# google-research/Splat-SLAM

Hardware: AMD Instinct MI355X
Metric: mapping frames/sec + render ms @640x480, 300k Gaussians; PSNR vs ref (higher is better)
Workload: dtype f32

## Files before the change

### include/splat_hip.h

```cpp
#ifndef SPLAT_HIP_H_
#define SPLAT_HIP_H_

#include <stddef.h>
#include <stdint.h>

#ifdef __cplusplus
extern "C" {
#endif

#define SGR_ABI_VERSION 10

typedef enum SgrStatus {
  SGR_OK = 0,
  SGR_ERR_INVALID = -1,
  SGR_ERR_WORKSPACE = -2,
  SGR_ERR_CAPACITY = -3,
  SGR_ERR_HIP = -4
} SgrStatus;

typedef struct SgrSettings {
  int32_t num_gaussians;
  int32_t image_height;
  int32_t image_width;
  int32_t sh_degree;
// ... 83 lines not shown
} SgrBackwardView;
int sgr_backward_views(int32_t num_views, const SgrBackwardView* views, const SgrInputs* in, const SgrGradInputs* grad_in,
                       void* stream);

int sgr_densify_stats(int64_t n, const float* dL_dmeans2D, const int32_t* radii, float* stat_grad_accum, float* stat_denom,
                      float* stat_max_radii, void* stream);

int sgr_query(const void* saved, int64_t* num_rendered_host, int32_t* overflow_host, void* stream);

int sgr_query_header(const void* saved, uint32_t words_host[16], void* stream);

int sgr_header_to_host(const void* saved, void* pinned_host64, void* stream);

int sgr_query_stats(const SgrWorkspace* ws, int32_t num_gaussians, int32_t image_height, int32_t image_width,
                    const int32_t* radii, int64_t stats_host[4], void* stream);
int sgr_query_depth_keys(const SgrWorkspace* ws, int32_t num_gaussians, int32_t image_height, int32_t image_width,
                         const int32_t* radii, float* depth_out, void* stream);
int sgr_query_list_histogram(const SgrWorkspace* ws, int32_t num_gaussians, int32_t image_height, int32_t image_width,
                             int64_t hist_host[8], void* stream);

#define SGR_OPT_FUSED_BLEND 0
#define SGR_OPT_UPSTREAM_POSE_JACOBIAN 1
#define SGR_OPT_SEGMENT_TEST 2
#define SGR_OPT_COUNT 3
int sgr_set_option(int32_t option, int32_t value);
int sgr_get_option(int32_t option);

#define SGR_PROFILE_KINDS 7
int sgr_profile_enable(uint32_t kind_mask);
int sgr_profile_read(float ms_host[SGR_PROFILE_KINDS], int64_t launches_host[SGR_PROFILE_KINDS]);

int sgr_mapping_loss(int32_t H, int32_t W, const float* image, const float* depth,
                     const float* gt_image, const float* gt_depth,
                     const float* exposure_a, const float* exposure_b,
                     float alpha, float rgb_boundary_threshold, float upstream,
                     float* loss, float* dL_dimage, float* dL_ddepth, float* dL_dexp_a, float* dL_dexp_b,
                     void* scratch, size_t scratch_bytes, void* stream);

size_t sgr_ssim_scratch_bytes(int32_t B, int32_t C, int32_t H, int32_t W);
int sgr_ssim(int32_t B, int32_t C, int32_t H, int32_t W, const float* img1, const float* img2, float* ssim_out, float* maps,
             void* scratch, size_t scratch_bytes, void* stream);
int sgr_ssim_backward(int32_t B, int32_t C, int32_t H, int32_t W, const float* img1, const float* img2, const float* maps,
                      const float* upstream, int32_t upstream_stride, float upstream_scale, float* dL_dimg1, void* stream);

typedef struct SgrMetricFrame {
  const float* render;
  const float* gt_image;
// ... 485 lines not shown
```

### splat_slam_amd/_native.py

```python
import ctypes as C
import os

_HERE = os.path.dirname(os.path.abspath(__file__))
LIB_PATH = os.environ.get("SPLAT_HIP_LIB") or os.path.join(_HERE, "lib", "libsplat_hip.so")

SGR_OPT_FUSED_BLEND = 0
SGR_OPT_UPSTREAM_POSE_JACOBIAN = 1
SGR_OPT_SEGMENT_TEST = 2
SGR_OK, SGR_ERR_INVALID, SGR_ERR_WORKSPACE, SGR_ERR_CAPACITY, SGR_ERR_HIP = 0, -1, -2, -3, -4

_fp = C.c_void_p


class SgrSettings(C.Structure):
    _fields_ = [("num_gaussians", C.c_int32), ("image_height", C.c_int32), ("image_width", C.c_int32),
                ("sh_degree", C.c_int32), ("sh_coeffs", C.c_int32), ("tanfovx", C.c_float), ("tanfovy", C.c_float),
                ("scale_modifier", C.c_float), ("prefiltered", C.c_int32), ("debug", C.c_int32),
                ("bg", _fp), ("viewmatrix", _fp), ("projmatrix", _fp), ("projmatrix_raw", _fp), ("campos", _fp)]


class SgrInputs(C.Structure):
    _fields_ = [("means3D", _fp), ("opacities", _fp), ("shs", _fp), ("colors_precomp", _fp), ("scales", _fp),
                ("rotations", _fp), ("cov3D_precomp", _fp)]


class SgrOutputs(C.Structure):
    _fields_ = [("color", _fp), ("depth", _fp), ("opacity", _fp), ("radii", _fp), ("n_touched", _fp)]


class SgrWorkspace(C.Structure):
    _fields_ = [("saved", _fp), ("saved_bytes", C.c_size_t), ("scratch", _fp), ("scratch_bytes", C.c_size_t),
# ... 350 lines not shown
```

### splat_slam_amd/csrc/sgr_api.hip

```cpp
#include <cstdarg>
#include <cstdio>
#include <cstring>
#include <cstdlib>
#include <vector>

#include <hip/hip_runtime.h>

#include "sgr_common.h"

namespace sgr {

void launch_preprocess_fwd(const ViewTab&, int, const LOff&, const Common&, const SgrInputs&, hipStream_t);
void launch_preprocess_bwd(const ViewTab&, int, const LOff&, const Common&, const SgrInputs&, const SgrGradInputs&, const FusedAdam*,
                           hipStream_t, bool mapping_loop = false);
void launch_binning(const ViewTab&, int, const LOff&, hipStream_t);
void launch_zero_heads(const ViewTab&, int, const LOff&, size_t, hipStream_t);
void launch_blend_fwd(const ViewTab&, int, const LOff&, const float*, const LossTab*, const LossCoef*, hipStream_t);
void launch_blend_bwd(const ViewTab&, int, const LOff&, const float*, const LossTab*, const LossCoef*, hipStream_t);
void launch_blend_fused(const ViewTab&, int, const LOff&, const float*, const LossTab&, const LossCoef&, hipStream_t);
bool blend_can_fuse(const LOff&);

static int g_opt[SGR_OPT_COUNT] = {1, 0, 0};

static thread_local char g_err[512] = "";
int set_error(int code, const char* fmt, ...) {
  va_list ap;
  va_start(ap, fmt);
  vsnprintf(g_err, sizeof(g_err), fmt, ap);
  va_end(ap);
  return code;
}
#define HIP_TRY(expr)                                                                                   \
  do {                                                                                                  \
    hipError_t _e = (expr);                                                                             \
    if (_e != hipSuccess) return set_error(SGR_ERR_HIP, "%s failed: %s", #expr, hipGetErrorString(_e)); \
  } while (0)

int debug_flags() {
  static int f = -1;
  if (f < 0) { const char* e = getenv("SGR_DEBUG"); f = e ? atoi(e) : 0; }
  return f | (g_opt[SGR_OPT_SEGMENT_TEST] ? 0 : 4);
}

static Layout make_layout(int N, int H, int W, int64_t cap) { return Layout(N, H, W, cap); }

// ... 268 lines not shown
  for (int base = 0; base < num_views; base += kMaxViews) {
    const int nv = num_views - base < kMaxViews ? num_views - base : kMaxViews;
    ViewTab tab = {};
    for (int v = 0; v < nv; ++v) {
      const SgrBackwardView& m = views[base + v];
      if (int rc = check_workspace(&m.ws, L)) return rc;
      tab_set_view(tab, v, &m.settings, nullptr, &m.ws);
      tab.radii[v] = const_cast<int32_t*>(m.radii);
      tab.dL_dcolor[v] = m.dL_dcolor; tab.dL_ddepth[v] = m.dL_ddepth; tab.dL_dtau[v] = m.dL_dtau; tab.dL_dmeans2D[v] = m.dL_dmeans2D;
    }
    SgrGradInputs gv = g;
    gv.accumulate = (grad_in->accumulate || base > 0) ? 1 : 0;
    launch_blend_bwd(tab, nv, d, f.settings.bg, nullptr, nullptr, st);
    launch_preprocess_bwd(tab, nv, d, cm, *in, gv, nullptr, st);
  }
  HIP_TRY(hipGetLastError());
  return SGR_OK;
}

}

static int map_views_impl(int32_t num_views, const SgrMapView* views, const SgrInputs* in, const SgrGradInputs* grads, float alpha,
                          float rgb_boundary_threshold, int32_t forward_only, FusedAdam* fused, bool* fused_done,
                          void* stream, bool store_sinks = false, const SgrSsimTerm* term = nullptr) {
  if (fused_done) *fused_done = false;
  if (num_views < 0 || (num_views > 0 && (!views || !in)) || (!forward_only && !grads))
    return set_error(SGR_ERR_INVALID, "map_views: null argument");
  if (num_views == 0) return SGR_OK;
  if (forward_only) term = nullptr;
  if (term) {
    if (!term->arena || term->max_views <= 0)
      return set_error(SGR_ERR_INVALID, "map_views: SSIM term without an arena");
    for (int v = 0; v < num_views; ++v) {
      const SgrMapView& m = views[v];
      const int H = m.settings.image_height, W = m.settings.image_width;
      if (!m.out.color || !m.out.depth || !m.out.opacity)
        return set_error(SGR_ERR_INVALID, "map_views: the SSIM loss needs every view's rendered image, depth and opacity");
      if (term->arena_bytes < sgr_ssim_term_bytes(term->max_views, H, W))
        return set_error(SGR_ERR_WORKSPACE, "map_views: SSIM arena too small (need %zu for %d views of %dx%d)",
                         sgr_ssim_term_bytes(term->max_views, H, W), term->max_views, W, H);
      if (!m.loss_scratch || m.loss_scratch_bytes < (size_t)ssim_loss_nparts(H, W) * sizeof(LossPart))
        return set_error(SGR_ERR_WORKSPACE, "map_views: loss_scratch too small for the SSIM loss (need %zu)",
                         (size_t)ssim_loss_nparts(H, W) * sizeof(LossPart));
    }
  }
  hipStream_t st = (hipStream_t)stream;
  bool uniform = true;
// ... 33 lines not shown
                                           mv.loss, mv.dL_dimage, mv.dL_ddepth, mv.dL_dexposure,
                                           mv.dL_dexposure ? mv.dL_dexposure + 1 : nullptr, stream))
          return rc;
      } else if (int rc = sgr_mapping_loss(mv.settings.image_height, mv.settings.image_width, mv.out.color, mv.out.depth, mv.gt_image,
                                           mv.gt_depth, mv.exposure_a, mv.exposure_b, alpha, rgb_boundary_threshold, 1.0f, mv.loss,
                                           mv.dL_dimage, mv.dL_ddepth, mv.dL_dexposure, mv.dL_dexposure ? mv.dL_dexposure + 1 : nullptr,
                                           mv.loss_scratch, mv.loss_scratch_bytes, stream)) {
        return rc;
      }
      SgrGradOutputs go = {mv.dL_dimage, mv.dL_ddepth};
      SgrGradInputs gi = *grads;
      gi.dL_dtau = mv.dL_dtau;
      if (int rc = sgr_backward(&mv.settings, in, mv.out.radii, &go, &gi, &mv.ws, stream)) return rc;
    }
    return SGR_OK;
  }
  Layout L = make_layout(f.settings.num_gaussians, f.settings.image_height, f.settings.image_width, f.ws.capacity);
  LOff d = L.dev();
  int hint = 0;
  for (int v = 0; v < num_views; ++v) hint = views[v].ws.max_list_hint > hint ? views[v].ws.max_list_hint : hint;
  d.set_hint(hint);
  Common cm = make_common(&f.settings);
  const int HW = f.settings.image_height * f.settings.image_width;
  for (int base = 0; base < num_views; base += kMaxViews) {
    const int nv = num_views - base < kMaxViews ? num_views - base : kMaxViews;
    ViewTab tab = {};
    LossTab lt = {};
    bool all_clean = true;
    for (int v = 0; v < nv; ++v) {
      const SgrMapView& m = views[base + v];
      all_clean = all_clean && m.ws.counters_clean != 0;
      if (int rc = check_workspace(&m.ws, L)) return rc;
      const bool no_images = !m.out.color && !m.out.depth && !m.out.opacity && !forward_only;
      if ((!no_images && (!m.out.color || !m.out.depth || !m.out.opacity)) || !m.out.radii)
        return set_error(SGR_ERR_INVALID, "map_views: null output pointer");
      tab_set_view(tab, v, &m.settings, &m.out, &m.ws);
      if (!forward_only) {
        if (!m.gt_image || !m.gt_depth || !m.dL_dimage || !m.dL_ddepth || !m.loss_scratch ||
            m.loss_scratch_bytes < (size_t)L.ntiles * sizeof(LossPart))
          return set_error(SGR_ERR_INVALID, "map_views: loss buffers missing (loss_scratch needs 16 B per 8x8 tile = %zu)",
                           (size_t)L.ntiles * sizeof(LossPart));
        tab.dL_dcolor[v] = m.dL_dimage; tab.dL_ddepth[v] = m.dL_ddepth; tab.dL_dtau[v] = m.dL_dtau;
        lt.image[v] = m.out.color; lt.depth[v] = m.out.depth; lt.gt_image[v] = m.gt_image; lt.gt_depth[v] = m.gt_depth;
        lt.exp_a[v] = m.exposure_a; lt.exp_b[v] = m.exposure_b; lt.loss[v] = m.loss; lt.dimage[v] = m.dL_dimage;
        lt.ddepth[v] = m.dL_ddepth; lt.da[v] = m.dL_dexposure; lt.db[v] = m.dL_dexposure ? m.dL_dexposure + 1 : nullptr;
        lt.parts[v] = m.loss_scratch;
      }
    }
    if (int rc = forward_batch(tab, nv, L, cm, *in, st, all_clean, d.mean_hint)) return rc;
    if (forward_only) {
      launch_blend_fwd(tab, nv, d, f.settings.bg, nullptr, nullptr, st);
      continue;
    }
    LossCoef lc = {alpha / (3.f * (float)HW), (1.f - alpha) / (float)HW, rgb_boundary_threshold};
    const bool fused_blend = !term && g_opt[SGR_OPT_FUSED_BLEND] != 0 && blend_can_fuse(d);
    int nparts = L.ntiles;
    if (term) {
      const int H = f.settings.image_height, W = f.settings.image_width;
      launch_blend_fwd(tab, nv, d, f.settings.bg, nullptr, nullptr, st);
      for (int g0 = 0; g0 < nv; g0 += term->max_views)
        launch_ssim_mapping_loss(lt, g0, nv - g0 < term->max_views ? nv - g0 : term->max_views, H, W, alpha, term->lambda_dssim,
                                 rgb_boundary_threshold, 1.f, (float*)term->arena, st);
      nparts = ssim_loss_nparts(H, W);
    } else if (fused_blend) {
      launch_blend_fused(tab, nv, d, f.settings.bg, lt, lc, st);
    } else {
      launch_blend_fwd(tab, nv, d, f.settings.bg, &lt, &lc, st);
    }
    const bool fuse = fused && num_views <= kMaxViews;
    if (fuse) {
      fused->tail_views = nv; fused->tail_nparts = nparts;
      fused->tail_inv_rgb = 1.f / (3.f * (float)HW); fused->tail_inv_dep = 1.f / (float)HW; fused->tail_alpha = alpha;
      for (int v = 0; v < nv; ++v) {
        fused->tail_parts[v] = lt.parts[v]; fused->tail_loss[v] = lt.loss[v]; fused->tail_da[v] = lt.da[v]; fused->tail_db[v] = lt.db[v];
      }
    } else {
      launch_mapping_loss_final(lt, nv, HW, nparts, alpha, st);
    }
    if (term) launch_blend_bwd(tab, nv, d, f.settings.bg, nullptr, nullptr, st);
    else if (!fused_blend) launch_blend_bwd(tab, nv, d, f.settings.bg, &lt, &lc, st);
    launch_preprocess_bwd(tab, nv, d, cm, *in, *grads, fuse ? fused : nullptr, st, true);
    if (fuse && fused_done) *fused_done = true;
  }
  HIP_TRY(hipGetLastError());
  return SGR_OK;
}

extern "C" {

int sgr_map_views(int32_t num_views, const SgrMapView* views, const SgrInputs* in, const SgrGradInputs* grads, float alpha,
                  float rgb_boundary_threshold, int32_t forward_only, void* stream) {
  return map_views_impl(num_views, views, in, grads, alpha, rgb_boundary_threshold, forward_only, nullptr, nullptr, stream);
}

}

static int map_step_impl(const SgrMapStep* p, bool skip_activate, bool grads_clean, bool allow_fuse, bool* fused_out, void* stream,
                         const SgrSsimTerm* term = nullptr) {
  if (fused_out) *fused_out = false;
  if (!p) return set_error(SGR_ERR_INVALID, "map_step: null argument");
  const bool adam_only = p->num_views == 0 && p->adam_groups;
  if (!skip_activate && !adam_only && (p->scaling || p->rotation || p->opacity))
    if (int rc = sgr_activate(p->num_gaussians, p->scaling, p->rotation, p->opacity, p->scales_out, p->rot_out, p->opac_out, stream)) return rc;
  FusedAdam fa;
  bool try_fuse = false;
  if (allow_fuse && p->adam_groups && p->num_views > 0 && p->num_views <= kMaxViews && !p->forward_only && p->grads && p->in && p->views) {
    const SgrGradInputs& g = *p->grads;
    const SgrAdamGroup* G = p->adam_groups;
    try_fuse = g.accumulate && g.dL_dmeans3D == G[0].grad && g.dL_dshs == G[1].grad && g.dL_dopacities == G[2].grad &&
               g.dL_dscales == G[3].grad && g.dL_drotations == G[4].grad && !g.dL_dmeans2D && !g.dL_dcolors_precomp &&
               !g.dL_dcov3D_precomp && p->in->shs && !p->in->colors_precomp && p->in->scales && p->in->rotations &&
               p->num_gaussians == p->views[0].settings.num_gaussians;
    for (int v = 0; v < p->num_views && try_fuse; ++v)
      try_fuse = !p->views[v].dL_dtau && p->views[v].settings.sh_degree == 0 && p->views[v].settings.sh_coeffs == 1;
    if (try_fuse) {
      if (int rc = make_fused_adam(p->num_gaussians, G, p->beta1, p->beta2, p->eps, p->iso_weight, &fa)) return rc;
      fa.grads_clean = grads_clean ? 1 : 0;
      fa.s_out = p->scales_out; fa.r_out = p->rot_out; fa.o_out = p->opac_out;
      fa.stat_accum = g.stat_grad_accum;
      fa.stat_denom = g.stat_grad_accum ? g.stat_denom : nullptr;
      fa.stat_maxr = g.stat_grad_accum ? g.stat_max_radii : nullptr;
// ... 14 lines not shown
               p->in->scales && p->in->rotations && p->num_gaussians == p->views[0].settings.num_gaussians;
    for (int v = 0; v < p->num_views && try_fuse; ++v)
      try_fuse = !p->views[v].dL_dtau && p->views[v].settings.sh_degree == 0 && p->views[v].settings.sh_coeffs == 1;
    if (try_fuse) {
      fa = FusedAdam{};
      fa.gather_only = p->grads_clean == -3 ? 2 : 1;
      fa.G.g[0].grad = g.dL_dmeans3D; fa.G.g[1].grad = g.dL_dshs; fa.G.g[2].grad = g.dL_dopacities;
      fa.G.g[3].grad = g.dL_dscales; fa.G.g[4].grad = g.dL_drotations;
      fa.stat_accum = g.stat_grad_accum;
      fa.stat_denom = g.stat_grad_accum ? g.stat_denom : nullptr;
      fa.stat_maxr = g.stat_grad_accum ? g.stat_max_radii : nullptr;
      if (p->exp_rows > 0) {
        if (!p->exp_param || !p->exp_grad || !p->exp_avg || !p->exp_avg_sq || !p->exp_step || !p->exp_active || p->exp_row_width <= 0)
          return set_error(SGR_ERR_INVALID, "map_step: exposure block incomplete");
        fa.exp_rows = p->exp_rows; fa.exp_width = p->exp_row_width; fa.exp_param = p->exp_param; fa.exp_grad = p->exp_grad;
        fa.exp_avg = p->exp_avg; fa.exp_avg_sq = p->exp_avg_sq; fa.exp_step = p->exp_step; fa.exp_active = p->exp_active;
        fa.exp_lr = p->exp_lr; fa.exp_b1 = p->exp_beta1; fa.exp_b2 = p->exp_beta2; fa.exp_eps = p->exp_eps;
      }
    }
  }
  bool fused = false;
  if (p->num_views > 0)
    if (int rc = map_views_impl(p->num_views, p->views, p->in, p->grads, p->alpha, p->rgb_boundary_threshold, p->forward_only,
                                try_fuse ? &fa : nullptr, &fused, stream, p->grads_clean == -3 && !p->adam_groups, term))
      return rc;
  if (p->adam_groups && !fused)
    if (int rc = gaussian_adam_step_act(p->num_gaussians, p->adam_groups, p->beta1, p->beta2, p->eps, p->iso_weight,
                                        adam_only && p->scaling ? p->scales_out : nullptr,
                                        adam_only && p->rotation ? p->rot_out : nullptr,
                                        adam_only && p->opacity ? p->opac_out : nullptr, stream))
      return rc;
  if (p->exp_rows > 0 && !fused)
    if (int rc = sgr_masked_adam(p->exp_rows, p->exp_row_width, p->exp_param, p->exp_grad, p->exp_avg, p->exp_avg_sq, p->exp_step,
                                 p->exp_active, p->exp_lr, p->exp_beta1, p->exp_beta2, p->exp_eps, stream))
      return rc;
  if (fused_out) *fused_out = fused;
  return SGR_OK;
}

extern "C" {

int sgr_map_step(const SgrMapStep* p, void* stream) {
  if (!p) return set_error(SGR_ERR_INVALID, "map_step: null argument");
  return map_step_impl(p, false, p->grads_clean > 0, p->grads_clean >= 0, nullptr, stream);
}

int sgr_map_step_ssim(const SgrMapStep* p, const SgrSsimTerm* term, void* stream) {
  if (!p) return set_error(SGR_ERR_INVALID, "map_step: null argument");
  return map_step_impl(p, false, p->grads_clean > 0, p->grads_clean >= 0, nullptr, stream, term);
}

}

static int map_run_impl(const SgrMapRun* r, const SgrSsimTerm* term, void* stream) {
  if (!r || r->num_iters < 0 || r->num_window < 0 || r->picks_per_iter < 0 || (r->num_window > 0 && !r->window) ||
      (r->picks_per_iter > 0 && (!r->pool || !r->picks || r->pool_size <= 0)))
    return set_error(SGR_ERR_INVALID, "map_run: bad argument");
  const int nv = r->num_window + r->picks_per_iter;
  if (nv > 64) return set_error(SGR_ERR_INVALID, "map_run: more than 64 views per iteration");
  SgrMapView views[64];
  for (int v = 0; v < r->num_window; ++v) views[v] = r->window[v];
  std::vector<char> pool_used((size_t)(r->pool_size > 0 ? r->pool_size : 0), 0);
  std::vector<char> slot_used((size_t)(r->picks_per_iter > 0 ? r->picks_per_iter : 0), 0);
  SgrMapStep st = r->step;
  st.views = views;
  st.num_views = nv;
  st.adam_groups = r->adam_groups;
  const int32_t exp_rows = st.exp_rows;
  bool prev_fused = false;
  for (int it = 0; it < r->num_iters; ++it) {
    for (int j = 0; j < r->picks_per_iter; ++j) {
      const int32_t k = r->picks[(size_t)it * r->picks_per_iter + j];
      if (k < 0 || k >= r->pool_size) return set_error(SGR_ERR_INVALID, "map_run: pick %d outside the pool", k);
      views[r->num_window + j] = r->pool[k];
      if (r->pick_ws) {
        views[r->num_window + j].ws = r->pick_ws[j];
        if (slot_used[j]) views[r->num_window + j].ws.counters_clean = 1;
        slot_used[j] = 1;
      } else if (pool_used[k]) {
        views[r->num_window + j].ws.counters_clean = 1;
      }
      pool_used[k] = 1;
    }
    if (it == 1)
      for (int v = 0; v < r->num_window; ++v) views[v].ws.counters_clean = 1;
    if (r->n_touched_last_only) {
      const bool last = it == r->num_iters - 1;
      for (int v = 0; v < r->num_window; ++v) views[v].out.n_touched = last ? r->window[v].out.n_touched : nullptr;
      if (!last)
        for (int j = 0; j < r->picks_per_iter; ++j) views[r->num_window + j].out.n_touched = nullptr;
    }
    if (r->adam_groups) {
      if (r->lr0) r->adam_groups[0].lr = r->lr0[it];
      for (int g = 0; g < 5; ++g)
        if (!r->adam_groups[g].skip) r->adam_groups[g].step += 1;
    }
    if (r->pool_exp_row && r->picks_per_iter > 0 && exp_rows > 0) {
      const int32_t row = r->pool_exp_row[r->picks[(size_t)it * r->picks_per_iter]];
      const size_t o = (size_t)(row < 0 ? 0 : row) * (size_t)st.exp_row_width;
      st.exp_rows = row < 0 ? 0 : 1;
      st.exp_param = r->step.exp_param + o; st.exp_grad = r->step.exp_grad + o;
      st.exp_avg = r->step.exp_avg + o; st.exp_avg_sq = r->step.exp_avg_sq + o;
      st.exp_step = r->step.exp_step + (row < 0 ? 0 : row);
    }
    bool fused = false;
    if (int rc = map_step_impl(&st, prev_fused, it == 0 ? r->step.grads_clean > 0 : r->adam_groups != nullptr, r->step.grads_clean >= 0,
                               &fused, stream, term))
      return rc;
    prev_fused = fused;
  }
  return SGR_OK;
}

extern "C" {

int sgr_map_run(const SgrMapRun* r, void* stream) { return map_run_impl(r, nullptr, stream); }
int sgr_map_run_ssim(const SgrMapRun* r, const SgrSsimTerm* term, void* stream) { return map_run_impl(r, term, stream); }

int sgr_query_stats(const SgrWorkspace* ws, int32_t N, int32_t H, int32_t W, const int32_t* radii, int64_t stats_host[4],
                    void* stream) {
  if (!ws || !ws->saved || !ws->scratch || !stats_host) return set_error(SGR_ERR_INVALID, "null argument");
  Layout L = make_layout(N, H, W, ws->capacity);
  hipStream_t st = (hipStream_t)stream;
  unsigned long long* d = (unsigned long long*)ws->scratch;
  HIP_TRY(hipMemsetAsync(d, 0, 32, st));
  hipLaunchKernelGGL(stats_kernel, dim3(64), dim3(256), 0, st, N, L.ntiles, radii, (const uint2*)((char*)ws->saved + L.o_ranges),
                     (const uint32_t*)((char*)ws->saved + L.o_tile_maxc), d);
  unsigned long long h[4];
  HIP_TRY(hipMemcpyAsync(h, d, 32, hipMemcpyDeviceToHost, st));
  HIP_TRY(hipStreamSynchronize(st));
// ... 79 lines not shown
```

### splat_slam_amd/csrc/sgr_aux.hip

```cpp
#include <cmath>

#include <cstdint>

#include "sgr_common.h"

namespace sgr {
int set_error(int code, const char* fmt, ...);


__global__ void __launch_bounds__(256) mapping_loss_kernel(LossTab tab, int HW, float w_rgb, float w_dep, float thr) {
  const int vw = blockIdx.y;
  const float* __restrict__ image = tab.image[vw];
  const float* __restrict__ depth = tab.depth[vw];
  const float* __restrict__ gt_image = tab.gt_image[vw];
  const float* __restrict__ gt_depth = tab.gt_depth[vw];
  float* __restrict__ dimage = tab.dimage[vw];
  float* __restrict__ ddepth = tab.ddepth[vw];
  LossPart* __restrict__ parts = (LossPart*)tab.parts[vw];
  const float ea = tab.exp_a[vw] ? __expf(tab.exp_a[vw][0]) : 1.f;
  const float eb = tab.exp_b[vw] ? tab.exp_b[vw][0] : 0.f;
  LossPart acc = {0.f, 0.f, 0.f, 0.f};
  for (int p = blockIdx.x * blockDim.x + threadIdx.x; p < HW; p += gridDim.x * blockDim.x) {
    float g0 = gt_image[p], g1 = gt_image[HW + p], g2 = gt_image[2 * HW + p];
    bool m = (g0 + g1 + g2) > thr;
// ... 314 lines not shown
      }
    }
    return;
  }
  __shared__ const char* s_scratch[kMaxViews];
  __shared__ const int32_t* s_radii[kMaxViews];
  __shared__ uint32_t s_over[kMaxViews];
#pragma unroll
  for (int u = 0; u < kMaxViews; ++u)
    if ((int)threadIdx.x == u && u < nviews) {
      s_scratch[u] = tab.scratch[u];
      s_radii[u] = tab.radii[u];
      s_over[u] = ((const SavedHeader*)tab.saved[u])->overflow;
    }
  __syncthreads();
  uint32_t truncated = 0u;
  for (int u = 0; u < nviews; ++u) truncated |= (s_over[u] != 0u ? 1u : 0u) << u;
  const int i = ((int)blockIdx.x - fa.tail_views) * blockDim.x + threadIdx.x;
  if (i >= L.N) return;
  float a[14];
#pragma unroll
  for (int k = 0; k < 14; ++k) a[k] = 0.f;
  float st_norm = 0.f, st_cnt = 0.f, st_maxr = 0.f;
  uint32_t seen = 0u;
  for (int p = 0; p < min(L.k1_parts, nviews); ++p) seen |= ((const uint32_t*)(tab.saved[0] + L.o_vismask))[(size_t)p * L.N + i];
  seen &= ~truncated;
  const bool any = seen != 0u;
  while (seen) {
    const int v = __builtin_ctz(seen);
    seen &= seen - 1u;
    const float4* rec = (const float4*)(s_scratch[v] + L.o_gradrec) + (size_t)i * 4;
    const int r = s_radii[v][i];
    float4 r0 = rec[0], r1 = rec[1], r2 = rec[2], r3 = rec[3];
    a[0] += r0.x; a[1] += r0.y; a[2] += r0.z; a[3] += r0.w; a[4] += r1.x; a[5] += r1.y; a[6] += r1.z; a[7] += r1.w;
    a[8] += r2.x; a[9] += r2.y; a[10] += r2.z; a[11] += r2.w; a[12] += r3.x; a[13] += r3.y;
    st_norm += sqrtf(r3.z * r3.z + r3.w * r3.w);
    st_cnt += 1.f;
    st_maxr = fmaxf(st_maxr, (float)r);
  }
  if (any && fa.stat_accum) {
    fa.stat_accum[i] += st_norm;
    fa.stat_denom[i] += st_cnt;
    fa.stat_maxr[i] = fmaxf(fa.stat_maxr[i], st_maxr);
  }
  if (MODE == 3) {
    if (!any) return;
    float* g0 = fa.G.g[0].grad + 3 * (size_t)i; float* g1 = fa.G.g[1].grad + 3 * (size_t)i; float* g3 = fa.G.g[3].grad + 3 * (size_t)i;
    float* g4 = fa.G.g[4].grad + 4 * (size_t)i;
    g0[0] += a[0]; g0[1] += a[1]; g0[2] += a[2];
    g1[0] += a[3]; g1[1] += a[4]; g1[2] += a[5];
    fa.G.g[2].grad[i] += a[6];
    g3[0] += a[7]; g3[1] += a[8]; g3[2] += a[9];
    g4[0] += a[10]; g4[1] += a[11]; g4[2] += a[12]; g4[3] += a[13];
    return;
  }
  if (MODE == 4) {
    st3(fa.G.g[0].grad + 3 * (size_t)i, F3{a[0], a[1], a[2]});
    st3(fa.G.g[1].grad + 3 * (size_t)i, F3{a[3], a[4], a[5]});
    fa.G.g[2].grad[i] = a[6];
    st3(fa.G.g[3].grad + 3 * (size_t)i, F3{a[7], a[8], a[9]});
    *(float4*)(fa.G.g[4].grad + 4 * (size_t)i) = make_float4(a[10], a[11], a[12], a[13]);
// ... 533 lines not shown
```

### splat_slam_amd/csrc/sgr_common.h

```cpp
#pragma once

#include <hip/hip_runtime.h>
#include <stdint.h>

#include "../../include/splat_hip.h"

namespace sgr {

constexpr float kNearPlane = 0.001f;
constexpr float kAlphaMin = 1.0f / 255.0f;
constexpr float kAlphaMax = 0.99f;
constexpr float kTEps = 1e-4f;
constexpr float kDilation = 0.3f;
constexpr float kTouchedT = 0.5f;
constexpr int kRefTile = 16;
constexpr int kTile = 8;
constexpr int kWave = 64;
constexpr int kCntSlotWords = 8;
constexpr uint32_t kTileCountLimit = 0xff00u;
__host__ __device__ inline size_t tile_counter_word(int x, int y, int gxp) { return ((size_t)(y >> 1) * gxp + (x >> 1)) * (kCntSlotWords / 2); }
__host__ __device__ inline int tile_counter_shift(int x, int y) { return 16 * ((y & 1) * 2 + (x & 1)); }
constexpr int kK1MaxParts = 4;
#ifndef SGR_K1_DENSE_PARTS
#define SGR_K1_DENSE_PARTS 2
// ... 210 lines not shown
  float* loss[kMaxViews];
  float* dimage[kMaxViews];
  float* ddepth[kMaxViews];
  float* da[kMaxViews];
  float* db[kMaxViews];
  void* parts[kMaxViews];
};
void launch_mapping_loss(const LossTab& tab, int nviews, int HW, float alpha, float thr, float upstream, hipStream_t st);
void launch_mapping_loss_final(const LossTab& tab, int nviews, int HW, int nparts, float alpha, hipStream_t st);
struct LossPart { float rgb, dep, da, db; };
size_t ssim_term_view_maps(int H, int W);
int ssim_loss_nparts(int H, int W);
void launch_ssim_mapping_loss(const LossTab& lt, int v0, int nv, int H, int W, float alpha, float lam, float thr, float upstream,
                              float* maps, hipStream_t st);
struct LossCoef { float w_rgb, w_dep, thr; };

struct AdamConst { float b1, b2, eps; float bc2_sqrt[5], step_size[5]; };
struct AdamGroups { SgrAdamGroup g[5]; int64_t r0[5], r1[5]; };
struct FusedAdam {
  AdamGroups G;
  AdamConst c;
  float iso_coef;
  int grads_clean;
  int gather_only;
  float *s_out, *r_out, *o_out;
  float *stat_accum, *stat_denom, *stat_maxr;
  int tail_views, tail_nparts;
  float tail_inv_rgb, tail_inv_dep, tail_alpha;
  const void* tail_parts[kMaxViews];
  float* tail_loss[kMaxViews];
  float* tail_da[kMaxViews];
  float* tail_db[kMaxViews];
  int exp_rows, exp_width;
  float* exp_param; const float* exp_grad; float* exp_avg; float* exp_avg_sq; int32_t* exp_step; const int32_t* exp_active;
  float exp_lr, exp_b1, exp_b2, exp_eps;
};
int make_fused_adam(int64_t n, const SgrAdamGroup groups[5], float beta1, float beta2, float eps, float iso_weight, FusedAdam* out);
int gaussian_adam_step_act(int64_t n, const SgrAdamGroup groups[5], float beta1, float beta2, float eps, float iso_weight,
                           float* s_out, float* r_out, float* o_out, void* stream);
void launch_gather_adam(const ViewTab& tab, int nviews, const LOff& L, const FusedAdam& fa, hipStream_t st);

enum ProfKind { PK_PRE_FWD = 0, PK_SCAN, PK_SCATTER, PK_BLEND_FUSED, PK_BLEND_FWD, PK_BLEND_BWD, PK_PRE_BWD };
void prof_begin(int kind, hipStream_t st);
void prof_end(int kind, hipStream_t st);
struct ProfScope {
  int kind; hipStream_t st;
  ProfScope(int k, hipStream_t s) : kind(k), st(s) { prof_begin(kind, st); }
  ~ProfScope() { prof_end(kind, st); }
};

__device__ __forceinline__ uint32_t abs_offset(const char* saved, const LOff& L, uint32_t g, uint32_t rel_offset) {
  return rel_offset + ((const uint32_t*)(saved + L.o_block_base_t))[g >> kSegShift];
}
__device__ __forceinline__ const GRec* grec_of(const char* saved, const LOff& L) { return (const GRec*)(saved + L.o_grec); }

struct __attribute__((packed, aligned(4))) F3 { float x, y, z; };
__device__ __forceinline__ F3 ld3(const float* p) { return *(const F3*)p; }
__device__ __forceinline__ void st3(float* p, F3 v) { *(F3*)p = v; }

struct V3 { float x, y, z; };
__device__ __forceinline__ V3 cross(V3 a, V3 b) {
  return {a.y * b.z - a.z * b.y, a.z * b.x - a.x * b.z, a.x * b.y - a.y * b.x};
}

template <int CTRL, int ROW_MASK = 0xf, int BANK_MASK = 0xf>
__device__ __forceinline__ float dpp_f(float old, float v) {
  return __builtin_bit_cast(float, __builtin_amdgcn_update_dpp(__builtin_bit_cast(int, old),
                                                                __builtin_bit_cast(int, v), CTRL, ROW_MASK,
                                                                BANK_MASK, false));
}
constexpr int DPP_ROW_SHR1 = 0x111, DPP_ROW_SHR2 = 0x112, DPP_ROW_SHR4 = 0x114, DPP_ROW_SHR8 = 0x118;
constexpr int DPP_WAVE_SHR1 = 0x138, DPP_ROW_BCAST15 = 0x142, DPP_ROW_BCAST31 = 0x143;

__device__ __forceinline__ float wave_scan_add(float v) {
  v += dpp_f<DPP_ROW_SHR1>(0.f, v);
  v += dpp_f<DPP_ROW_SHR2>(0.f, v);
  v += dpp_f<DPP_ROW_SHR4>(0.f, v);
  v += dpp_f<DPP_ROW_SHR8>(0.f, v);
// ... 55 lines not shown
```

### splat_slam_amd/csrc/sgr_preprocess.hip

```cpp
#include "sgr_common.h"

namespace sgr {

struct Cam {
  float vm[16];
  float pm[16];
};

__device__ __forceinline__ void load16(const float* __restrict__ src, float* dst) {
#pragma unroll
  for (int i = 0; i < 16; ++i) dst[i] = src[i];
}

__device__ __forceinline__ void quat_to_R(const float q[4], float R[3][3]) {
  float r = q[0], x = q[1], y = q[2], z = q[3];
  R[0][0] = 1.f - 2.f * (y * y + z * z); R[0][1] = 2.f * (x * y - r * z); R[0][2] = 2.f * (x * z + r * y);
  R[1][0] = 2.f * (x * y + r * z); R[1][1] = 1.f - 2.f * (x * x + z * z); R[1][2] = 2.f * (y * z - r * x);
  R[2][0] = 2.f * (x * z - r * y); R[2][1] = 2.f * (y * z + r * x); R[2][2] = 1.f - 2.f * (x * x + y * y);
}

__device__ __forceinline__ void cov3d_from_scale_rot(const float s[3], float mod, const float q[4], float S6[6]) {
  float R[3][3];
  quat_to_R(q, R);
  float M[3][3];
// ... 352 lines not shown
            const float yz0 = fminf(fminf(v0[1] * iz0, v0[1] * iz1), fminf(v1[1] * iz0, v1[1] * iz1));
            const float yz1 = fmaxf(fmaxf(v0[1] * iz0, v0[1] * iz1), fmaxf(v1[1] * iz0, v1[1] * iz1));
            const float limx = 1.3f * cm.tanfovx, limy = 1.3f * cm.tanfovy;
            const float tn = (fx * fx * (1.f + limx * limx) + fy * fy * (1.f + limy * limy)) * iz0 * iz0;
            const float rad = ceilf(3.f * sqrtf(tn * tsm * 1.01f + 1.0f)) + 3.f;
            const float ox = 0.5f * L.W * (p_projraw[tid][8] + 1.f) - 0.5f, oy = 0.5f * L.H * (p_projraw[tid][9] + 1.f) - 0.5f;
            const float px0 = fx * xz0 + ox - rad - 1.f, px1 = fx * xz1 + ox + rad + (kRefTile - 1) + 1.f;
            const float py0 = fy * yz0 + oy - rad - 1.f, py1 = fy * yz1 + oy + rad + (kRefTile - 1) + 1.f;
            if (isfinite(px0) && isfinite(px1) && isfinite(py0) && isfinite(py1) && isfinite(rad))
              maybe = !(px1 < 0.f || py1 < 0.f || px0 >= (float)(L.sgx * kRefTile) || py0 >= (float)(L.sgy * kRefTile));
          }
        }
        if (maybe) atomicOr(&seg_views, 1u << tid);
      }
      __syncthreads();
    }
    const uint32_t segv = seg_views;
    const float sroot = __builtin_amdgcn_sqrtf(fmaxf(trS, 0.f)) * 1.0005f;
#pragma unroll 2
    for (int v = 0; v < nviews; ++v) {
      bool pass = false;
      if (ia < N && (v % nparts) == part) {
        if (!(L.dbg & 16)) {
        p_radii[v][ia] = 0;
        if (p_ntouched[v]) p_ntouched[v][ia] = 0;
        }
        if (L.dbg & 2) pass = (p[0] + trS == 12345.678f);
        else if (segv & (1u << v)) pass = (L.dbg & 8) ? maybe_visible(p, trS, L.H, L.W, cm.tanfovx, cm.tanfovy, mats[v], mats[v] + 16, L.sgx, L.sgy)
                                                      : maybe_visible_planes(p, sroot, mats[v], mats[v] + 16, cullK[v], L.H, L.W, L.sgx, L.sgy);
      }
      const unsigned long long m = __ballot(pass);
      if (lane == 0) wtot[v][wv] = (uint32_t)__popcll(m);
      if (pass) {
        passbits |= 1u << v;
        ranks[v >> 2] |= (uint32_t)__popcll(m & ((1ull << lane) - 1ull)) << ((v & 3) * 8);
      }
    }
  }
  __syncthreads();
  if (tid == 0) {
    uint32_t run = 0;
    for (int v = 0; v < nviews; ++v) {
      vstart[v] = run;
      run += wtot[v][0] + wtot[v][1] + wtot[v][2] + wtot[v][3];
    }
    for (int v = nviews; v <= kMaxViews; ++v) vstart[v] = run;
  }
// ... 27 lines not shown
      PreIn in;
      { const F3 t = ld3(means3D + 3 * i); in.p[0] = t.x; in.p[1] = t.y; in.p[2] = t.z; }
      in.opac = opacities[i];
      if (cov3D_precomp) {
#pragma unroll
        for (int k = 0; k < 6; ++k) in.S6[k] = cov3D_precomp[6 * i + k];
      } else {
        const F3 sc3 = ld3(scales + 3 * i);
        const float4 q4 = *(const float4*)(rotations + 4 * i);
        float s_in[3] = {sc3.x, sc3.y, sc3.z};
        float q_in[4] = {q4.x, q4.y, q4.z, q4.w};
        cov3d_from_scale_rot(s_in, cm.mod, q_in, in.S6);
      }
      in.c_in[0] = in.c_in[1] = in.c_in[2] = 0.f;
      if (colors_precomp) { in.c_in[0] = colors_precomp[3 * i]; in.c_in[1] = colors_precomp[3 * i + 1]; in.c_in[2] = colors_precomp[3 * i + 2]; }
      else if (cm.deg == 0) { in.c_in[0] = shs[(size_t)i * cm.M * 3]; in.c_in[1] = shs[(size_t)i * cm.M * 3 + 1]; in.c_in[2] = shs[(size_t)i * cm.M * 3 + 2]; }
      preprocess_view(in, i, L.H, L.W, cm.deg, cm.M, cm.tanfovx, cm.tanfovy, vm, pm, p_campos[v], shs,
                      colors_precomp != nullptr, L.gx, L.gy, L.sgx, L.sgy, o);
    }
    const uint32_t cnt = o.visible ? (uint32_t)((o.x1 - o.x0) * (o.y1 - o.y0)) : 0u;
    const uint32_t vis = o.visible ? 1u : 0u;
    if (o.visible && !(L.dbg & 128)) {
      atomicOr(&vis_bits[i - seg0], 1u << v);
      p_radii[v][i] = (int32_t)o.rad;
      float4* rec = (float4*)((GRec*)(saved + L.o_grec) + i);
      rec[0] = make_float4(o.px, o.py, __uint_as_float((uint32_t)o.x0 | ((uint32_t)o.y0 << 16)),
                           __uint_as_float((uint32_t)o.x1 | ((uint32_t)o.y1 << 16)));
      rec[1] = make_float4(o.A, o.B, o.C, o.opac);
      rec[2] = make_float4(o.rgb[0], o.rgb[1], o.rgb[2], o.depth);
    }
    const uint32_t my_rx = (uint32_t)o.x0 | ((uint32_t)o.x1 << 16), my_ry = (uint32_t)o.y0 | ((uint32_t)o.y1 << 16);
    const uint32_t nops = cnt > 0u ? (uint32_t)((((o.x1 - 1) >> 1) - (o.x0 >> 1) + 1) * (((o.y1 - 1) >> 1) - (o.y0 >> 1) + 1)) : 0u;
    op_rect[tid] = make_uint4(my_rx, my_ry, (uint32_t)v, (uint32_t)i);
    op_depth[tid] = __float_as_uint(o.depth);
    Footprint my_foot{0.f, 0.f, 0.f, 0.f, 0.f, 0.f, 0.f, -1.f};
    if (o.visible && footprint_worthwhile(o.x1 - o.x0, o.y1 - o.y0)) my_foot = make_footprint(o.px, o.py, o.A, o.B, o.C, o.opac, 0.005f);
    op_foot[tid][0] = make_float4(my_foot.px, my_foot.py, my_foot.A, my_foot.B);
    op_foot[tid][1] = make_float4(my_foot.C, my_foot.invA, my_foot.invC, my_foot.thr);
    auto op_geom = [](uint32_t rx, uint32_t ry, int k, const Footprint& foot) -> uint32_t {
      const int x0 = (int)(rx & 0xffffu), x1 = (int)(rx >> 16), y0 = (int)(ry & 0xffffu), y1 = (int)(ry >> 16);
      const int per_row = ((x1 - 1) >> 1) - (x0 >> 1) + 1;
      int q = (int)(((float)k + 0.5f) * __builtin_amdgcn_rcpf((float)per_row));
      int rem = k - q * per_row;
      if (rem < 0) { --q; rem += per_row; }
      if (rem >= per_row) { ++q; rem -= per_row; }
      const int bx = ((x0 >> 1) + rem) * 2, by = ((y0 >> 1) + q) * 2;
      const bool c0 = bx >= x0, c1 = bx + 1 < x1, r0 = by >= y0, r1 = by + 1 < y1;
// ... 340 lines not shown
      }
      float r = q[0], x = q[1], y = q[2], z = q[3];
      g_q[0] = 2.f * (-z * dR[0][1] + y * dR[0][2] + z * dR[1][0] - x * dR[1][2] - y * dR[2][0] + x * dR[2][1]);
      g_q[1] = 2.f * (y * dR[0][1] + z * dR[0][2] + y * dR[1][0] - 2.f * x * dR[1][1] - r * dR[1][2] + z * dR[2][0] + r * dR[2][1] - 2.f * x * dR[2][2]);
      g_q[2] = 2.f * (-2.f * y * dR[0][0] + x * dR[0][1] + r * dR[0][2] + x * dR[1][0] + z * dR[1][2] - r * dR[2][0] + z * dR[2][1] - 2.f * y * dR[2][2]);
      g_q[3] = 2.f * (-2.f * z * dR[0][0] - r * dR[0][1] + x * dR[0][2] + r * dR[1][0] - 2.f * z * dR[1][1] + y * dR[1][2] + x * dR[2][0] + y * dR[2][1]);
    }
  }
  (void)dcolors;
#pragma unroll
  for (int k = 0; k < 3; ++k) { acc.p[k] += g_p[k]; acc.s[k] += g_s[k]; acc.rgb_or_sh0[k] += sh0[k]; }
#pragma unroll
  for (int k = 0; k < 4; ++k) acc.q[k] += g_q[k];
#pragma unroll
  for (int k = 0; k < 6; ++k) acc.S6[k] += g_S6[k];
  acc.op += g_op;
  acc.m2[0] = g_m2[0]; acc.m2[1] = g_m2[1];
}

template <int LPG>
__global__ void __launch_bounds__(256) __attribute__((amdgpu_waves_per_eu(3, 8))) preprocess_bwd_dense_kernel(
    ViewTab tab, LOff L, Common cm, const float* __restrict__ means3D, const float* __restrict__ shs,
    const float* __restrict__ colors_precomp, const float* __restrict__ scales, const float* __restrict__ rotations,
    const float* __restrict__ cov3D_precomp, float* __restrict__ dshs, float* __restrict__ dcov3D, int accumulate) {
  const int v = blockIdx.y;
  const char* saved = tab.saved[v];
  const int V = (int)((const SavedHeader*)(saved + L.o_hdr))->num_visible;
  constexpr int kPerBlock = 256 / LPG;
  if ((int)(blockIdx.x * kPerBlock) >= V) return;
  const int t = blockIdx.x * kPerBlock + (int)threadIdx.x / LPG;
  const bool have = t < V;
  const int i = have ? (int)((const uint32_t*)(saved + L.o_vis_list))[t] : 0;
  uint4 q3 = make_uint4(0u, 0u, 0u, 0u);
  float4 g0 = make_float4(0.f, 0.f, 0.f, 0.f), g1 = g0;
  if (have) {
    const float4* rec = (const float4*)(grec_of(saved, L) + i);
    g0 = rec[0]; g1 = rec[1]; q3 = ((const uint4*)rec)[3];
  }
  const uint32_t my_r01 = __float_as_uint(g0.z), my_r23 = __float_as_uint(g0.w);
  const bool tested = have && footprint_worthwhile((int)(my_r23 & 0xffffu) - (int)(my_r01 & 0xffffu), (int)(my_r23 >> 16) - (int)(my_r01 >> 16));
  const Footprint foot = tested ? make_footprint(g0.x, g0.y, g1.x, g1.y, g1.z, g1.w, 0.006f)
                                : Footprint{0.f, 0.f, 0.f, 0.f, 0.f, 0.f, 0.f, -1.f};
  auto slot_unwritten = [](const Footprint& f, uint32_t r01, uint32_t r23, uint32_t k) -> bool {
    if (!(f.thr >= 0.f)) return false;
    const int x0 = (int)(r01 & 0xffffu), y0 = (int)(r01 >> 16), w = (int)(r23 & 0xffffu) - x0;
    int q = (int)(((float)k + 0.5f) * __builtin_amdgcn_rcpf((float)w));
    int rem = (int)k - q * w;
// ... 133 lines not shown
  }
  if (!have || (LPG > 1 && (threadIdx.x & (LPG - 1)) != 0)) return;
  {
    const float G0 = gsum[0], G1 = gsum[1], Gxx = gsum[2], Gxy = gsum[3], Go = gsum[4], Gr = gsum[5], Gg = gsum[6], Gb = gsum[7],
                Gyy = gsum[8], Gd = gsum[9];
    gsum[0] = (-(g1.x * G0) - g1.y * G1) * (0.5f * (float)L.W);
    gsum[1] = (-(g1.z * G1) - g1.y * G0) * (0.5f * (float)L.H);
    gsum[2] = -0.5f * Gxx;
    gsum[3] = -Gxy;
    gsum[4] = -0.5f * Gyy;
    gsum[5] = Go; gsum[6] = Gr; gsum[7] = Gg; gsum[8] = Gb; gsum[9] = Gd;
  }
  float tau[6] = {0.f, 0.f, 0.f, 0.f, 0.f, 0.f};
  GaussGrad acc;
#pragma unroll
  for (int j = 0; j < 3; ++j) { acc.p[j] = 0.f; acc.s[j] = 0.f; acc.rgb_or_sh0[j] = 0.f; }
#pragma unroll
  for (int j = 0; j < 4; ++j) acc.q[j] = 0.f;
#pragma unroll
  for (int j = 0; j < 6; ++j) acc.S6[j] = 0.f;
  acc.op = 0.f; acc.m2[0] = 0.f; acc.m2[1] = 0.f;
  preprocess_bwd_one_view(i, L.H, L.W, cm.deg, cm.M, cm.tanfovx, cm.tanfovy, cm.mod, tab.viewmatrix[v], tab.projmatrix[v],
                          tab.projraw[v], tab.campos[v], means3D, shs, colors_precomp, scales, rotations, cov3D_precomp,
                          gsum, q3.w, dshs, accumulate, acc, tau, cm.upstream_pose_jac);
  float4* rec = (float4*)(tab.scratch[v] + L.o_gradrec) + (size_t)i * 4;
  rec[0] = make_float4(acc.p[0], acc.p[1], acc.p[2], acc.rgb_or_sh0[0]);
  rec[1] = make_float4(acc.rgb_or_sh0[1], acc.rgb_or_sh0[2], acc.op, acc.s[0]);
  rec[2] = make_float4(acc.s[1], acc.s[2], acc.q[0], acc.q[1]);
  rec[3] = make_float4(acc.q[2], acc.q[3], acc.m2[0], acc.m2[1]);
  if (float* m2 = tab.dL_dmeans2D[v]) {
    if (((const SavedHeader*)(saved + L.o_hdr))->overflow == 0u) {
      m2[3 * (size_t)i] = acc.m2[0];
      m2[3 * (size_t)i + 1] = acc.m2[1];
    }
  }
  if (dcov3D) {
#pragma unroll
    for (int j = 0; j < 6; ++j) { if (accumulate) dcov3D[6 * i + j] += acc.S6[j]; else dcov3D[6 * i + j] = acc.S6[j]; }
  }
  if (tab.dL_dtau[v]) {
    float* tr = (float*)(tab.scratch[v] + L.o_taurec) + (size_t)t * 6;
#pragma unroll
    for (int j = 0; j < 6; ++j) tr[j] = tau[j];
  }
}

__global__ void __launch_bounds__(256) grad_gather_kernel(
    ViewTab tab, int nviews, LOff L, int deg, int M, int has_colors, float* __restrict__ dmeans3D,
    float* __restrict__ dmeans2D, float* __restrict__ dopac, float* __restrict__ dshs, float* __restrict__ dcolors,
    float* __restrict__ dscales, float* __restrict__ drots, float* __restrict__ dcov3D, int accumulate,
    float* __restrict__ stat_accum, float* __restrict__ stat_denom, float* __restrict__ stat_maxr) {
  __shared__ float red[4][6];
// ... 83 lines not shown
  for (int b = lane; b < nblk; b += 64) acc += tau_part[(size_t)b * 6 + k];
  red[k][lane] = acc;
  __syncthreads();
  if (lane == 0) {
    float t = 0.f;
    for (int l = 0; l < 64; ++l) t += red[k][l];
    dtau[k] = t;
  }
}

void launch_preprocess_fwd(const ViewTab& tab, int nviews, const LOff& L, const Common& cm, const SgrInputs& in, hipStream_t st) {
  if (L.N <= 0) return;
  ProfScope prof(PK_PRE_FWD, st);
  hipLaunchKernelGGL(preprocess_fwd_kernel, dim3(L.nseg, min(L.k1_parts, nviews)), dim3(256), 0, st, tab, nviews, L, cm, in.means3D, in.opacities,
                     in.shs, in.colors_precomp, in.scales, in.rotations, in.cov3D_precomp);
}

void launch_preprocess_bwd(const ViewTab& tab, int nviews, const LOff& L, const Common& cm, const SgrInputs& in,
                           const SgrGradInputs& g, const FusedAdam* fused, hipStream_t st, bool mapping_loop) {
  if (L.N <= 0) return;
  ProfScope prof(PK_PRE_BWD, st);
  static const int forced = []() { const char* e = getenv("SGR_DENSE_QUAD"); return e ? atoi(e) : -1; }();
  const bool quad = forced >= 0 ? forced != 0 : (mapping_loop && nviews == 1);
  if (quad)
    hipLaunchKernelGGL(preprocess_bwd_dense_kernel<4>, dim3(L.pre_blocks * 4, nviews), dim3(256), 0, st, tab, L, cm, in.means3D, in.shs,
                       in.colors_precomp, in.scales, in.rotations, in.cov3D_precomp, g.dL_dshs, g.dL_dcov3D_precomp, g.accumulate);
  else
    hipLaunchKernelGGL(preprocess_bwd_dense_kernel<1>, dim3(L.pre_blocks, nviews), dim3(256), 0, st, tab, L, cm, in.means3D, in.shs,
                       in.colors_precomp, in.scales, in.rotations, in.cov3D_precomp, g.dL_dshs, g.dL_dcov3D_precomp, g.accumulate);
  if (fused) {
    launch_gather_adam(tab, nviews, L, *fused, st);
    return;
  }
  hipLaunchKernelGGL(grad_gather_kernel, dim3(L.pre_blocks), dim3(256), 0, st, tab, nviews, L, cm.deg, cm.M,
                     in.colors_precomp != nullptr ? 1 : 0, g.dL_dmeans3D, g.dL_dmeans2D, g.dL_dopacities, g.dL_dshs,
                     g.dL_dcolors_precomp, g.dL_dscales, g.dL_drotations, g.dL_dcov3D_precomp, g.accumulate,
                     g.stat_grad_accum, (g.stat_grad_accum ? g.stat_denom : nullptr),
                     (g.stat_grad_accum ? g.stat_max_radii : nullptr));
  bool any_tau = false;
  for (int v = 0; v < nviews; ++v) any_tau = any_tau || tab.dL_dtau[v] != nullptr;
  if (any_tau) hipLaunchKernelGGL(tau_reduce_kernel, dim3(nviews), dim3(384), 0, st, tab, L);
}

}
```

Baseline: 62.13.

## Fold radius and grad norm into gradient record tail to skip radii gathers

The preprocess forward packs the integer screen radius into the upper bits of the saved clamp word. The backward kernel then writes the 2D-gradient norm and the unpacked radius into the last slot of the per-view gradient record, so the fused gather/Adam kernel no longer reads the separate radii array or recomputes the norm. The mapping loop also marks views whose radii output is never read later and skips writing it by nulling the pointer. This removes scattered radii loads and stores in the backward gather, at the cost of more cross-file bookkeeping and a packed radius encoding that loses precision for very large radii.

```diff
diff --git a/include/splat_hip.h b/include/splat_hip.h
--- a/include/splat_hip.h
+++ b/include/splat_hip.h
@@ -129,7 +129,9 @@
 #define SGR_OPT_FUSED_BLEND 0
 #define SGR_OPT_UPSTREAM_POSE_JACOBIAN 1
 #define SGR_OPT_SEGMENT_TEST 2
-#define SGR_OPT_COUNT 3
+#define SGR_OPT_TAIL_GATHERS 3
+#define SGR_TAIL_GATHERS_ALL 1
+#define SGR_OPT_COUNT 4
 int sgr_set_option(int32_t option, int32_t value);
 int sgr_get_option(int32_t option);
 
diff --git a/splat_slam_amd/_native.py b/splat_slam_amd/_native.py
--- a/splat_slam_amd/_native.py
+++ b/splat_slam_amd/_native.py
@@ -7,6 +7,8 @@
 SGR_OPT_FUSED_BLEND = 0
 SGR_OPT_UPSTREAM_POSE_JACOBIAN = 1
 SGR_OPT_SEGMENT_TEST = 2
+SGR_OPT_TAIL_GATHERS = 3
+SGR_TAIL_GATHERS_ALL = 1
 SGR_OK, SGR_ERR_INVALID, SGR_ERR_WORKSPACE, SGR_ERR_CAPACITY, SGR_ERR_HIP = 0, -1, -2, -3, -4
 
 _fp = C.c_void_p
diff --git a/splat_slam_amd/csrc/sgr_api.hip b/splat_slam_amd/csrc/sgr_api.hip
--- a/splat_slam_amd/csrc/sgr_api.hip
+++ b/splat_slam_amd/csrc/sgr_api.hip
@@ -20,7 +20,9 @@
 void launch_blend_fused(const ViewTab&, int, const LOff&, const float*, const LossTab&, const LossCoef&, hipStream_t);
 bool blend_can_fuse(const LOff&);
 
-static int g_opt[SGR_OPT_COUNT] = {1, 0, 0};
+static int g_opt[SGR_OPT_COUNT] = {1, 0, 0, 0};
+static const int g_tail_env = []() { if (const char* e = getenv("SGR_TAIL_GATHERS")) g_opt[SGR_OPT_TAIL_GATHERS] = atoi(e); return 0; }();
+static int tail_gathers() { return g_opt[SGR_OPT_TAIL_GATHERS]; }
 
 static thread_local char g_err[512] = "";
 int set_error(int code, const char* fmt, ...) {
@@ -335,7 +337,7 @@
 
 static int map_views_impl(int32_t num_views, const SgrMapView* views, const SgrInputs* in, const SgrGradInputs* grads, float alpha,
                           float rgb_boundary_threshold, int32_t forward_only, FusedAdam* fused, bool* fused_done,
-                          void* stream, bool store_sinks = false, const SgrSsimTerm* term = nullptr) {
+                          void* stream, bool store_sinks = false, const SgrSsimTerm* term = nullptr, uint64_t radii_unread = 0) {
   if (fused_done) *fused_done = false;
   if (num_views < 0 || (num_views > 0 && (!views || !in)) || (!forward_only && !grads))
     return set_error(SGR_ERR_INVALID, "map_views: null argument");
@@ -415,6 +417,9 @@
   d.set_hint(hint);
   Common cm = make_common(&f.settings);
   const int HW = f.settings.image_height * f.settings.image_width;
+  const bool fuse = fused && num_views <= kMaxViews;
+  const bool tail_rec = fuse && !forward_only && !tail_gathers() && !fused->gather_only;
+  if (fuse) fused->rec_tail = tail_rec ? 1 : 0;
   for (int base = 0; base < num_views; base += kMaxViews) {
     const int nv = num_views - base < kMaxViews ? num_views - base : kMaxViews;
     ViewTab tab = {};
@@ -428,6 +433,7 @@
       if ((!no_images && (!m.out.color || !m.out.depth || !m.out.opacity)) || !m.out.radii)
         return set_error(SGR_ERR_INVALID, "map_views: null output pointer");
       tab_set_view(tab, v, &m.settings, &m.out, &m.ws);
+      if (tail_rec && ((radii_unread >> (base + v)) & 1u)) tab.radii[v] = nullptr;
       if (!forward_only) {
         if (!m.gt_image || !m.gt_depth || !m.dL_dimage || !m.dL_ddepth || !m.loss_scratch ||
             m.loss_scratch_bytes < (size_t)L.ntiles * sizeof(LossPart))
@@ -460,7 +466,6 @@
     } else {
       launch_blend_fwd(tab, nv, d, f.settings.bg, &lt, &lc, st);
     }
-    const bool fuse = fused && num_views <= kMaxViews;
     if (fuse) {
       fused->tail_views = nv; fused->tail_nparts = nparts;
       fused->tail_inv_rgb = 1.f / (3.f * (float)HW); fused->tail_inv_dep = 1.f / (float)HW; fused->tail_alpha = alpha;
@@ -489,7 +494,7 @@
 }
 
 static int map_step_impl(const SgrMapStep* p, bool skip_activate, bool grads_clean, bool allow_fuse, bool* fused_out, void* stream,
-                         const SgrSsimTerm* term = nullptr) {
+                         const SgrSsimTerm* term = nullptr, uint64_t radii_unread = 0) {
   if (fused_out) *fused_out = false;
   if (!p) return set_error(SGR_ERR_INVALID, "map_step: null argument");
   const bool adam_only = p->num_views == 0 && p->adam_groups;
@@ -550,7 +555,7 @@
   bool fused = false;
   if (p->num_views > 0)
     if (int rc = map_views_impl(p->num_views, p->views, p->in, p->grads, p->alpha, p->rgb_boundary_threshold, p->forward_only,
-                                try_fuse ? &fa : nullptr, &fused, stream, p->grads_clean == -3 && !p->adam_groups, term))
+                                try_fuse ? &fa : nullptr, &fused, stream, p->grads_clean == -3 && !p->adam_groups, term, radii_unread))
       return rc;
   if (p->adam_groups && !fused)
     if (int rc = gaussian_adam_step_act(p->num_gaussians, p->adam_groups, p->beta1, p->beta2, p->eps, p->iso_weight,
@@ -596,7 +601,21 @@
   st.adam_groups = r->adam_groups;
   const int32_t exp_rows = st.exp_rows;
   bool prev_fused = false;
+  std::vector<int> last_pick((size_t)(r->pool_size > 0 ? r->pool_size : 0), -1);
+  for (int it = 0; it < r->num_iters; ++it)
+    for (int j = 0; j < r->picks_per_iter; ++j) {
+      const int32_t k = r->picks[(size_t)it * r->picks_per_iter + j];
+      if (k >= 0 && k < r->pool_size) last_pick[k] = it;
+    }
   for (int it = 0; it < r->num_iters; ++it) {
+    uint64_t radii_unread = 0;
+    if (r->n_touched_last_only) {
+      if (it != r->num_iters - 1) radii_unread = r->num_window >= 64 ? ~0ull : (1ull << r->num_window) - 1ull;
+      for (int j = 0; j < r->picks_per_iter; ++j) {
+        const int32_t k = r->picks[(size_t)it * r->picks_per_iter + j];
+        if (k >= 0 && k < r->pool_size && last_pick[k] > it) radii_unread |= 1ull << (r->num_window + j);
+      }
+    }
     for (int j = 0; j < r->picks_per_iter; ++j) {
       const int32_t k = r->picks[(size_t)it * r->picks_per_iter + j];
       if (k < 0 || k >= r->pool_size) return set_error(SGR_ERR_INVALID, "map_run: pick %d outside the pool", k);
@@ -633,7 +652,7 @@
     }
     bool fused = false;
     if (int rc = map_step_impl(&st, prev_fused, it == 0 ? r->step.grads_clean > 0 : r->adam_groups != nullptr, r->step.grads_clean >= 0,
-                               &fused, stream, term))
+                               &fused, stream, term, radii_unread))
       return rc;
     prev_fused = fused;
   }
diff --git a/splat_slam_amd/csrc/sgr_aux.hip b/splat_slam_amd/csrc/sgr_aux.hip
--- a/splat_slam_amd/csrc/sgr_aux.hip
+++ b/splat_slam_amd/csrc/sgr_aux.hip
@@ -360,6 +360,7 @@
 #pragma unroll
   for (int k = 0; k < 14; ++k) a[k] = 0.f;
   float st_norm = 0.f, st_cnt = 0.f, st_maxr = 0.f;
+  const bool rec_tail = fa.rec_tail != 0;
   uint32_t seen = 0u;
   for (int p = 0; p < min(L.k1_parts, nviews); ++p) seen |= ((const uint32_t*)(tab.saved[0] + L.o_vismask))[(size_t)p * L.N + i];
   seen &= ~truncated;
@@ -368,13 +369,14 @@
     const int v = __builtin_ctz(seen);
     seen &= seen - 1u;
     const float4* rec = (const float4*)(s_scratch[v] + L.o_gradrec) + (size_t)i * 4;
-    const int r = s_radii[v][i];
+    int r = 0;
+    if (!rec_tail) r = s_radii[v][i];
     float4 r0 = rec[0], r1 = rec[1], r2 = rec[2], r3 = rec[3];
     a[0] += r0.x; a[1] += r0.y; a[2] += r0.z; a[3] += r0.w; a[4] += r1.x; a[5] += r1.y; a[6] += r1.z; a[7] += r1.w;
     a[8] += r2.x; a[9] += r2.y; a[10] += r2.z; a[11] += r2.w; a[12] += r3.x; a[13] += r3.y;
-    st_norm += sqrtf(r3.z * r3.z + r3.w * r3.w);
+    st_norm += rec_tail ? r3.z : m2_norm(r3.z, r3.w);
     st_cnt += 1.f;
-    st_maxr = fmaxf(st_maxr, (float)r);
+    st_maxr = fmaxf(st_maxr, rec_tail ? r3.w : (float)r);
   }
   if (any && fa.stat_accum) {
     fa.stat_accum[i] += st_norm;
diff --git a/splat_slam_amd/csrc/sgr_common.h b/splat_slam_amd/csrc/sgr_common.h
--- a/splat_slam_amd/csrc/sgr_common.h
+++ b/splat_slam_amd/csrc/sgr_common.h
@@ -256,6 +256,7 @@
   AdamConst c;
   float iso_coef;
   int grads_clean;
+  int rec_tail;
   int gather_only;
   float *s_out, *r_out, *o_out;
   float *stat_accum, *stat_denom, *stat_maxr;
@@ -288,6 +289,22 @@
 }
 __device__ __forceinline__ const GRec* grec_of(const char* saved, const LOff& L) { return (const GRec*)(saved + L.o_grec); }
 
+__device__ __forceinline__ float m2_norm(float x, float y) {
+#pragma clang fp contract(off)
+  const float xx = x * x, yy = y * y;
+  return sqrtf(xx + yy);
+}
+
+__device__ __forceinline__ uint32_t pack_clamp_radius(uint32_t clamp_bits, float rad) {
+  const float f = (float)(int32_t)rad;
+  const uint32_t e = f < 268435456.f ? (uint32_t)f : (1u << 28) | (uint32_t)(f * 0.03125f);
+  return (clamp_bits & 7u) | (e << 3);
+}
+__device__ __forceinline__ float unpack_radius(uint32_t word) {
+  const uint32_t e = word >> 3;
+  return (e >> 28) ? (float)(e & 0x0fffffffu) * 32.f : (float)e;
+}
+
 struct __attribute__((packed, aligned(4))) F3 { float x, y, z; };
 __device__ __forceinline__ F3 ld3(const float* p) { return *(const F3*)p; }
 __device__ __forceinline__ void st3(float* p, F3 v) { *(F3*)p = v; }
diff --git a/splat_slam_amd/csrc/sgr_preprocess.hip b/splat_slam_amd/csrc/sgr_preprocess.hip
--- a/splat_slam_amd/csrc/sgr_preprocess.hip
+++ b/splat_slam_amd/csrc/sgr_preprocess.hip
@@ -398,7 +398,7 @@
       bool pass = false;
       if (ia < N && (v % nparts) == part) {
         if (!(L.dbg & 16)) {
-        p_radii[v][ia] = 0;
+        if (p_radii[v]) p_radii[v][ia] = 0;
         if (p_ntouched[v]) p_ntouched[v][ia] = 0;
         }
         if (L.dbg & 2) pass = (p[0] + trS == 12345.678f);
@@ -472,7 +472,8 @@
     const uint32_t vis = o.visible ? 1u : 0u;
     if (o.visible && !(L.dbg & 128)) {
       atomicOr(&vis_bits[i - seg0], 1u << v);
-      p_radii[v][i] = (int32_t)o.rad;
+      if (p_radii[v]) p_radii[v][i] = (int32_t)o.rad;
+      o.clamped = pack_clamp_radius(o.clamped, o.rad);
       float4* rec = (float4*)((GRec*)(saved + L.o_grec) + i);
       rec[0] = make_float4(o.px, o.py, __uint_as_float((uint32_t)o.x0 | ((uint32_t)o.y0 << 16)),
                            __uint_as_float((uint32_t)o.x1 | ((uint32_t)o.y1 << 16)));
@@ -859,7 +860,7 @@
 __global__ void __launch_bounds__(256) __attribute__((amdgpu_waves_per_eu(3, 8))) preprocess_bwd_dense_kernel(
     ViewTab tab, LOff L, Common cm, const float* __restrict__ means3D, const float* __restrict__ shs,
     const float* __restrict__ colors_precomp, const float* __restrict__ scales, const float* __restrict__ rotations,
-    const float* __restrict__ cov3D_precomp, float* __restrict__ dshs, float* __restrict__ dcov3D, int accumulate) {
+    const float* __restrict__ cov3D_precomp, float* __restrict__ dshs, float* __restrict__ dcov3D, int accumulate, int rec_tail) {
   const int v = blockIdx.y;
   const char* saved = tab.saved[v];
   const int V = (int)((const SavedHeader*)(saved + L.o_hdr))->num_visible;
@@ -1039,12 +1040,13 @@
   acc.op = 0.f; acc.m2[0] = 0.f; acc.m2[1] = 0.f;
   preprocess_bwd_one_view(i, L.H, L.W, cm.deg, cm.M, cm.tanfovx, cm.tanfovy, cm.mod, tab.viewmatrix[v], tab.projmatrix[v],
                           tab.projraw[v], tab.campos[v], means3D, shs, colors_precomp, scales, rotations, cov3D_precomp,
-                          gsum, q3.w, dshs, accumulate, acc, tau, cm.upstream_pose_jac);
+                          gsum, q3.w & 7u, dshs, accumulate, acc, tau, cm.upstream_pose_jac);
   float4* rec = (float4*)(tab.scratch[v] + L.o_gradrec) + (size_t)i * 4;
   rec[0] = make_float4(acc.p[0], acc.p[1], acc.p[2], acc.rgb_or_sh0[0]);
   rec[1] = make_float4(acc.rgb_or_sh0[1], acc.rgb_or_sh0[2], acc.op, acc.s[0]);
   rec[2] = make_float4(acc.s[1], acc.s[2], acc.q[0], acc.q[1]);
-  rec[3] = make_float4(acc.q[2], acc.q[3], acc.m2[0], acc.m2[1]);
+  if (rec_tail) rec[3] = make_float4(acc.q[2], acc.q[3], m2_norm(acc.m2[0], acc.m2[1]), unpack_radius(q3.w));
+  else rec[3] = make_float4(acc.q[2], acc.q[3], acc.m2[0], acc.m2[1]);
   if (float* m2 = tab.dL_dmeans2D[v]) {
     if (((const SavedHeader*)(saved + L.o_hdr))->overflow == 0u) {
       m2[3 * (size_t)i] = acc.m2[0];
@@ -1174,12 +1176,13 @@
   ProfScope prof(PK_PRE_BWD, st);
   static const int forced = []() { const char* e = getenv("SGR_DENSE_QUAD"); return e ? atoi(e) : -1; }();
   const bool quad = forced >= 0 ? forced != 0 : (mapping_loop && nviews == 1);
+  const int rec_tail = fused && fused->rec_tail ? 1 : 0;
   if (quad)
     hipLaunchKernelGGL(preprocess_bwd_dense_kernel<4>, dim3(L.pre_blocks * 4, nviews), dim3(256), 0, st, tab, L, cm, in.means3D, in.shs,
-                       in.colors_precomp, in.scales, in.rotations, in.cov3D_precomp, g.dL_dshs, g.dL_dcov3D_precomp, g.accumulate);
+                       in.colors_precomp, in.scales, in.rotations, in.cov3D_precomp, g.dL_dshs, g.dL_dcov3D_precomp, g.accumulate, rec_tail);
   else
     hipLaunchKernelGGL(preprocess_bwd_dense_kernel<1>, dim3(L.pre_blocks, nviews), dim3(256), 0, st, tab, L, cm, in.means3D, in.shs,
-                       in.colors_precomp, in.scales, in.rotations, in.cov3D_precomp, g.dL_dshs, g.dL_dcov3D_precomp, g.accumulate);
+                       in.colors_precomp, in.scales, in.rotations, in.cov3D_precomp, g.dL_dshs, g.dL_dcov3D_precomp, g.accumulate, rec_tail);
   if (fused) {
     launch_gather_adam(tab, nviews, L, *fused, st);
     return;
```

Result: faster. 64.27, median of 5 (+3.4%).
